# uuwee/Vulkan-PBR-Renderer

Hardware: AMD Instinct MI355X
Metric: IBL-prefilter Mtexels/s (specular prefilter all mips + irradiance; PBR-shaded Mpixels/s under extra.shade_c5 / extra.shade) (higher is better)
Workload: dtype f32; 1 GPU; C4: 4096x4096 specular prefilter (6 faces, 13 mips) + 128x128 irradiance from a 2048^2 HDR cube; env=procedural HDR cube 2048^2 x6 RGBA32F (seed 0x5eed0004, RGBE round-tripped), overlap=False, parallelism=single GPU

## Files before the change

### vulkan-pbr-renderer_amd/csrc/k_mc_region.hip

```cpp
#include "pbr_device.h"
#include "pbr_kernels.h"
#include "k_mc_internal.h"

#include <stdlib.h>
#include <mutex>
#include <type_traits>

typedef float v4f __attribute__((ext_vector_type(4)));
typedef const __attribute__((address_space(4))) v4f* ctab_t;
typedef const __attribute__((address_space(3))) v4f* lds_v4f_p;
typedef const __attribute__((address_space(4))) unsigned* cu32_t;

#define REG_MAX_S 16
#ifndef MC_HEAD_FIRST_SUB
#define MC_HEAD_FIRST_SUB 1
#endif
#ifndef MC_HEAD_FIRST_G1
#define MC_HEAD_FIRST_G1 1
#endif

#ifndef MC_TILE32_SUB
#define MC_TILE32_SUB 1
#endif
#ifndef MC_TILE32_MIN_SIZE
#define MC_TILE32_MIN_SIZE 1024
#endif

struct RegArgs {
    McArgs a;
    int G;
    int RC;
    int NR;
    int NW;
    int expect[REG_MAX_S];
    int pole_row[2];
    const unsigned* tabmax;
    int cut;
    int absorb;
    unsigned long long* stats;
};

__device__ __forceinline__ void face_coords(int f, float x, float y, float z, float& sc, float& tc, float& ma) {
    switch (f) {
    case 0: sc = -z; tc = -y; ma = x; break;
    case 1: sc = z; tc = -y; ma = -x; break;
    case 2: sc = x; tc = z; ma = y; break;
    case 3: sc = x; tc = -z; ma = -y; break;
    case 4: sc = x; tc = -y; ma = z; break;
    default: sc = -x; tc = -y; ma = -z; break;
    }
}

struct RegionView {
    unsigned lds_base;
    f3 Pb, Pt, Pr;
    float half_n, off;
    float ulo, uhi, vlo, vhi;
};

__device__ __forceinline__ void to_face(const v4f e, const RegionView& V, float& sc, float& tc, float& ma) {
    sc = fmaf(e.x, V.Pb.x, fmaf(e.y, V.Pt.x, e.z * V.Pr.x));
    tc = fmaf(e.x, V.Pb.y, fmaf(e.y, V.Pt.y, e.z * V.Pr.y));
    ma = fmaf(e.x, V.Pb.z, fmaf(e.y, V.Pt.z, e.z * V.Pr.z));
}

template <int CLS>
__device__ __forceinline__ void on_face(float sc, float tc, float ma, bool& c1, bool& c2) {
    if (CLS == 0) { c1 = ma > fabsf(sc); c2 = ma > fabsf(tc); }
    else if (CLS == 1) { c1 = ma >= fabsf(sc); c2 = ma > fabsf(tc); }
    else { c1 = ma >= fabsf(sc); c2 = ma >= fabsf(tc); }
}

template <int RS>
__device__ __forceinline__ void tap_accumulate(float w, float u, float v, unsigned lds_base, float& ar, float& ag, float& ab) {
    const int il = (int)u, jl = (int)v;
    const float a = __builtin_amdgcn_fractf(u), b = __builtin_amdgcn_fractf(v);
    unsigned t16, addr;
    asm("v_lshl_add_u32 %0, %1, 4, %2" : "=v"(t16) : "v"(il), "s"(lds_base));
    asm("v_mad_u32_u24 %0, %1, %2, %3" : "=v"(addr) : "v"(jl), "s"(RS * 16), "v"(t16));
    lds_v4f_p tp = (lds_v4f_p)(unsigned long long)addr;
    v4f q00 = tp[0], q10 = tp[1], q01 = tp[RS], q11 = tp[RS + 1];
    asm("" : "+v"(q00)); asm("" : "+v"(q10)); asm("" : "+v"(q01)); asm("" : "+v"(q11));
    const float wa = w * a;
    const float w11 = wa * b;
    const float w10 = wa - w11;
    const float wt = w - wa;
    const float w01 = wt * b;
    const float w00 = wt - w01;
    ar = fmaf(w11, q11.x, fmaf(w01, q01.x, fmaf(w10, q10.x, fmaf(w00, q00.x, ar))));
    ag = fmaf(w11, q11.y, fmaf(w01, q01.y, fmaf(w10, q10.y, fmaf(w00, q00.y, ag))));
    ab = fmaf(w11, q11.z, fmaf(w01, q01.z, fmaf(w10, q10.z, fmaf(w00, q00.z, ab))));
}

template <int RS, bool SUB, int CLS, bool ACC = true>
__device__ __forceinline__ void region_sample(const v4f e, const RegionView& V, float& ar, float& ag, float& ab, unsigned& cnt) {
    float sc, tc, ma;
    to_face(e, V, sc, tc, ma);
    bool c1, c2;
    on_face<CLS>(sc, tc, ma, c1, c2);
    unsigned long long inm = __builtin_amdgcn_ballot_w64(c1) & __builtin_amdgcn_ballot_w64(c2);
    if (inm == 0) return;
    if (!ACC && !SUB) { cnt += (unsigned)__builtin_popcountll(inm); return; }
    bool in = c1 && c2;
    const float h = __builtin_amdgcn_rcpf(ma) * V.half_n;
    const float u = fmaf(sc, h, V.off), v = fmaf(tc, h, V.off);
    if (SUB) {
        const bool c3 = u >= V.ulo, c4 = u < V.uhi, c5 = v >= V.vlo, c6 = v < V.vhi;
        inm &= __builtin_amdgcn_ballot_w64(c3) & __builtin_amdgcn_ballot_w64(c4) & __builtin_amdgcn_ballot_w64(c5) & __builtin_amdgcn_ballot_w64(c6);
        in = in && c3 && c4 && c5 && c6;
    }
    cnt += (unsigned)__builtin_popcountll(inm);
    if (ACC && in) tap_accumulate<RS>(e.w, u, v, V.lds_base, ar, ag, ab);
}

template <int RS>
__device__ __forceinline__ void certain_sample(const v4f e, const RegionView& V, float& ar, float& ag, float& ab) {
    float sc, tc, ma;
    to_face(e, V, sc, tc, ma);
    const float h = __builtin_amdgcn_rcpf(ma) * V.half_n;
    tap_accumulate<RS>(e.w, fmaf(sc, h, V.off), fmaf(tc, h, V.off), V.lds_base, ar, ag, ab);
}

template <int RS, bool SUB, int CLS, bool ACC = true>
__device__ __forceinline__ void lane_sample(const v4f e, const RegionView& V, float& ar, float& ag, float& ab, unsigned& cnt) {
    float sc, tc, ma;
    to_face(e, V, sc, tc, ma);
    bool c1, c2;
    on_face<CLS>(sc, tc, ma, c1, c2);
    bool in = c1 && c2;
    if (SUB && __builtin_amdgcn_ballot_w64(in) == 0ull) return;
    const float h = __builtin_amdgcn_rcpf(ma) * V.half_n;
    const float u = fmaf(sc, h, V.off), v = fmaf(tc, h, V.off);
    if (SUB) in = in && u >= V.ulo && u < V.uhi && v >= V.vlo && v < V.vhi;
    if (in) {
        cnt += 1u;
        if (ACC) tap_accumulate<RS>(e.w, u, v, V.lds_base, ar, ag, ab);
    }
}

template <typename F>
__device__ __forceinline__ void each_sample(unsigned m, ctab_t tw, F&& f) {
    if (m == 0u) return;
    v4f e = tw[__builtin_ctz(m)];
    m &= m - 1u;
    while (m) {
        const v4f en = tw[__builtin_ctz(m)];
        m &= m - 1u;
        f(e);
        e = en;
    }
    f(e);
}

__device__ __forceinline__ float absorb_threshold(float wmax, float m) {
    const float t = wmax * m * 1.00000095367431640625f * 0x1p25f;
    return t < 0x1p-100f ? 0x1p-100f : t;
}

__device__ __forceinline__ void count_absorbed(unsigned* skc, unsigned m, unsigned mu) {
    if (skc && (threadIdx.x & 63) == 0) {
        atomicAdd(&skc[0], 1u);
        atomicAdd(&skc[1], (unsigned)__builtin_popcount(m));
        atomicAdd(&skc[2], (unsigned)__builtin_popcount(mu));
    }
}

template <int RS, bool SUB, int CLS, int REG_S, bool CERT, bool LEAN>
__device__ __forceinline__ void region_pass(const RegionView& V, const unsigned* __restrict__ mwords, const unsigned* __restrict__ cwords, cu32_t wmg,
                                            unsigned rbits, unsigned* skc, int NW, int w0, int w1, ctab_t tab,
                                            float& ar, float& ag, float& ab, unsigned& cnt) {
    unsigned mnext = w0 < w1 ? (unsigned)__builtin_amdgcn_readfirstlane((int)mwords[w0]) : 0u;
    unsigned cnext = (CERT && w0 < w1) ? (unsigned)__builtin_amdgcn_readfirstlane((int)cwords[w0]) : 0u;
    for (int w = w0; w < w1; w += REG_S) {
        unsigned m = mnext;
        unsigned c = cnext;
        mnext = w + REG_S < w1 ? (unsigned)__builtin_amdgcn_readfirstlane((int)mwords[w + REG_S]) : 0u;
        if (CERT) {
            cnext = w + REG_S < w1 ? (unsigned)__builtin_amdgcn_readfirstlane((int)cwords[w + REG_S]) : 0u;
            cnt += 64u * (unsigned)__builtin_popcount(m & c);
        }
        ctab_t tw = tab + (w << 5);
        const unsigned wb = (rbits < 0x7f800000u && m != 0u) ? (LEAN ? wmg[w] : (unsigned)__builtin_amdgcn_readfirstlane((int)cwords[NW + w])) : 0x7f800000u;
        if (wb < 0x7f800000u) {
            const float T = absorb_threshold(__uint_as_float(wb), __uint_as_float(rbits));
            if (__builtin_amdgcn_ballot_w64(!(ar >= T && ag >= T && ab >= T)) == 0ull) {
                if (!CERT) {
                    c = (unsigned)__builtin_amdgcn_readfirstlane((int)cwords[w]);
                    cnt += 64u * (unsigned)__builtin_popcount(m & c);
                }
                count_absorbed(skc, m, m & ~c);
                m &= ~c;
                while (m) {
                    const int i0 = __builtin_ctz(m);
                    m &= m - 1u;
                    region_sample<RS, SUB, CLS, false>(tw[i0], V, ar, ag, ab, cnt);
                }
                continue;
            }
        }
        while (m) {
            const int i0 = __builtin_ctz(m);
            m &= m - 1u;
            const bool two = m != 0u;
            const int i1 = two ? __builtin_ctz(m) : i0;
            m &= m - 1u;
            const v4f e0 = tw[i0];
            const v4f e1 = tw[i1];
            if (CERT && ((c >> i0) & 1u)) certain_sample<RS>(e0, V, ar, ag, ab);
            else region_sample<RS, SUB, CLS>(e0, V, ar, ag, ab, cnt);
            if (two) {
                if (CERT && ((c >> i1) & 1u)) certain_sample<RS>(e1, V, ar, ag, ab);
                else region_sample<RS, SUB, CLS>(e1, V, ar, ag, ab, cnt);
            }
        }
    }
}

template <int RS, bool SUB, int CLS, int REG_S, bool CERT, bool LEAN>
__device__ __forceinline__ void region_pass_runs(const RegionView& V, const unsigned* __restrict__ mwords, const unsigned* __restrict__ cwords, cu32_t wmg,
                                                 unsigned rbits, unsigned* skc, int NW, int s, unsigned long long wsel, ctab_t tab,
                                                 float& ar, float& ag, float& ab, unsigned& cnt) {
    const int wl = s + REG_S * (int)(threadIdx.x & 63);
    unsigned long long nz = __builtin_amdgcn_ballot_w64(wl < NW && mwords[wl] != 0u) & wsel;
    auto tested = [&](const v4f e) { lane_sample<RS, SUB, CLS>(e, V, ar, ag, ab, cnt); };
    while (nz) {
        const int w = s + REG_S * (int)__builtin_ctzll(nz);
        nz &= nz - 1ull;
        const unsigned m = (unsigned)__builtin_amdgcn_readfirstlane((int)mwords[w]);
        unsigned c = CERT ? (unsigned)__builtin_amdgcn_readfirstlane((int)cwords[w]) : 0u;
        ctab_t tw = tab + (w << 5);
        const unsigned wb = rbits < 0x7f800000u ? (LEAN ? wmg[w] : (unsigned)__builtin_amdgcn_readfirstlane((int)cwords[NW + w])) : 0x7f800000u;
        if (wb < 0x7f800000u) {
            const float T = absorb_threshold(__uint_as_float(wb), __uint_as_float(rbits));
            if (__builtin_amdgcn_ballot_w64(!(ar >= T && ag >= T && ab >= T)) == 0ull) {
                if (!CERT) c = (unsigned)__builtin_amdgcn_readfirstlane((int)cwords[w]);
                cnt += (unsigned)__builtin_popcount(m & c);
                count_absorbed(skc, m, m & ~c);
                each_sample(m & ~c, tw, [&](const v4f e) { lane_sample<RS, SUB, CLS, false>(e, V, ar, ag, ab, cnt); });
                continue;
            }
        }
        if (!CERT) { each_sample(m, tw, tested); continue; }
        cnt += (unsigned)__builtin_popcount(m & c);
        unsigned mc = m & c, mu = m & ~c;
        for (;;) {
            const unsigned below = mu ? (mu & (0u - mu)) - 1u : ~0u;
            each_sample(mc & below, tw, [&](const v4f e) { certain_sample<RS>(e, V, ar, ag, ab); });
            mc &= ~below;
            if (!mu) break;
            const int it = __builtin_ctz(mu);
            mu &= mu - 1u;
            tested(tw[it]);
        }
    }
}

template <bool LEAN, bool G1, bool TWO>
__device__ __forceinline__ void region_bin(unsigned* masks, unsigned* any, unsigned* dmax, int NR, int NW, int G, int RC, int n,
                                           f3 R, f3 T, f3 B, f3 Rc, f3 Tc, f3 Bc, ctab_t tab, int n_tab, int tid,
                                           unsigned* cmask, unsigned* wmax, int ntail, int lim, bool keep_cut, int head_end) {
    const float nf = (float)n;
    const float half_n = 0.5f * nf;
    const float off = 0.5f * nf + 0.5f;
    for (int k = tid; k < NR * NW + NR + 1 + ntail; k += 1024) masks[k] = 0u;
    __syncthreads();
    {
        f3 dR = sub3(R, Rc), dT = sub3(T, Tc), dB = sub3(B, Bc);
        float d2 = dot3(dR, dR) + dot3(dT, dT) + dot3(dB, dB);
        atomicMax(dmax, __float_as_uint(sqrtf(d2)));
    }
    __syncthreads();
    const float delta = __uint_as_float(*dmax) * 0.70710678f * 1.001f + 4e-6f;
    const int i_end = (TWO && !keep_cut) ? min(n_tab, lim) : n_tab;
    for (int i = tid; i < i_end; i += 1024) {
        const v4f e = tab[i];
        const int ab = TWO ? (i >= lim ? 2 : (i >= head_end ? 1 : 0)) : 0;
        const float Lx = fmaf(e.x, Bc.x, fmaf(e.y, Tc.x, e.z * Rc.x));
        const float Ly = fmaf(e.x, Bc.y, fmaf(e.y, Tc.y, e.z * Rc.y));
        const float Lz = fmaf(e.x, Bc.z, fmaf(e.y, Tc.z, e.z * Rc.z));
        const unsigned bit = 1u << (i & 31);
        if (!LEAN && wmax) atomicMax(&wmax[i >> 5], __float_as_uint(e.w));
#pragma unroll
        for (int f = 0; f < 6; ++f) {
            float sc, tc, ma;
            face_coords(f, Lx, Ly, Lz, sc, tc, ma);
            const float d2 = 1.41421357f * delta;
            if (!(ma + d2 >= fabsf(sc)) || !(ma + d2 >= fabsf(tc))) continue;
            int lo_u = 0, hi_u = n, lo_v = 0, hi_v = n;
            const float mlo = ma - delta;
            bool certain = false;
            if (mlo > 0.2f) {
                const float rm = LEAN ? __builtin_amdgcn_rcpf(ma) : 1.0f / ma, rl = LEAN ? __builtin_amdgcn_rcpf(mlo) : 1.0f / mlo;
                const float ru = sc * rm, rv = tc * rm;
                const float gu = (fabsf(sc) + delta) * rl, gv = (fabsf(tc) + delta) * rl;
                const float su = fmaf(gu, gu, 1.0f), sv = fmaf(gv, gv, 1.0f);
                const float mu = delta * (LEAN ? __builtin_amdgcn_sqrtf(su) : sqrtf(su)) * rl * half_n * 1.0001f + 0.05f;
                const float mv = delta * (LEAN ? __builtin_amdgcn_sqrtf(sv) : sqrtf(sv)) * rl * half_n * 1.0001f + 0.05f;
                const float uc = fmaf(ru, half_n, off), vc = fmaf(rv, half_n, off);
                const float ul = floorf(uc - mu), uh = floorf(uc + mu), vl = floorf(vc - mv), vh = floorf(vc + mv);
                if (uh < 0.0f || ul > nf || vh < 0.0f || vl > nf) continue;
                lo_u = (int)fmaxf(ul, 0.0f); hi_u = (int)fminf(uh, nf);
                lo_v = (int)fmaxf(vl, 0.0f); hi_v = (int)fminf(vh, nf);
                certain = cmask && ma - d2 > fabsf(sc) && ma - d2 > fabsf(tc) && ul >= 0.0f && uh <= nf && vl >= 0.0f && vh <= nf;
            }
            if (LEAN && G1) {
                if (certain) atomicOr(&cmask[i >> 5], bit);
                atomicOr(&masks[f * NW + (i >> 5)], bit);
                if (TWO) ((unsigned char*)any)[4 * f + ab] = 1;
                else any[f] = 1u;
                continue;
            }
            const int rc = LEAN ? 65 : RC;
            const int gx0 = lo_u / rc, gx1 = hi_u / rc, gy0 = lo_v / rc, gy1 = hi_v / rc;
            if (certain && gx0 == gx1 && gy0 == gy1) atomicOr(&cmask[i >> 5], bit);
            for (int gy = gy0; gy <= gy1; ++gy)
                for (int gx = gx0; gx <= gx1; ++gx) {
                    const int r = (f * G + gy) * G + gx;
                    atomicOr(&masks[r * NW + (i >> 5)], bit);
                    if (TWO) ((unsigned char*)any)[4 * r + ab] = 1;
                    else any[r] = 1u;
                }
        }
    }
}

__device__ __forceinline__ void tile_of_block(const RegArgs& q, int& face, int& tx, int& ty) {
    const McArgs& p = q.a;
    const unsigned tile = blockIdx.x;
    face = p.face0 + (int)(tile / (unsigned)p.tiles_per_face);
    const int tf = (int)(tile % (unsigned)p.tiles_per_face);
    ty = tf / p.tiles_x;
    tx = tf % p.tiles_x;
    if (face < 2) {
        const int ny = p.tiles_per_face / p.tiles_x, pr = q.pole_row[face];
        const int a = min(pr, ny - 1 - pr);
        if (ty <= 2 * a) { const int h = (ty + 1) >> 1; ty = (ty & 1) ? pr + h : pr - h; }
        else { const int rest = ty - 2 * a; ty = (pr > ny - 1 - pr) ? pr - a - rest : pr + a + rest; }
    }
}

template <int TILE>
__device__ __forceinline__ void texel_of_thread(const McArgs& p, int tx, int ty, int t, int& x, int& y) {
    constexpr int QW = TILE / 8, QSH = TILE == 32 ? 2 : 1;
    static_assert(QW == 1 << QSH, "TILE is 16 or 32");
    const int q8 = t >> 6, l8 = t & 63;
    x = tx * TILE + (q8 & (QW - 1)) * 8 + (l8 & 7);
    y = p.y0 + ty * TILE + (q8 >> QSH) * 8 + (l8 >> 3);
}

template <int REG_S, bool RUNS>
__device__ __forceinline__ unsigned cut_credit(int cw, int NW, int n_tab) {
    const int last = NW - 1, kc = (last - cw) / REG_S + 1;
    if (cw > last) return 0u;
    return (unsigned)(32 * kc - ((last - cw) % REG_S == 0 ? 32 * NW - n_tab : 0)) * (RUNS ? 1u : 64u);
}

template <int RS>
__device__ __forceinline__ void stage_rows(float4* region, const float4* __restrict__ fsrc, int nb, int rcx, int rcy, int tid) {
    int tid_s = tid;
    asm volatile("" : "+v"(tid_s));
    const int wv = __builtin_amdgcn_readfirstlane(tid_s >> 6), ln = tid_s & 63;
    const unsigned cx = (unsigned)min(ln, rcx) << 4;
    const char* const base = (const char*)fsrc;
    const unsigned rowb = (unsigned)nb << 4;
    const float4 v0 = *(const float4*)(base + (size_t)((unsigned)min(wv, rcy) * rowb) + cx);
    const float4 v1 = *(const float4*)(base + (size_t)((unsigned)min(wv + 16, rcy) * rowb) + cx);
    const float4 v2 = *(const float4*)(base + (size_t)((unsigned)min(wv + 32, rcy) * rowb) + cx);
    const float4 v3 = *(const float4*)(base + (size_t)((unsigned)min(wv + 48, rcy) * rowb) + cx);
    const float4 v4 = *(const float4*)(base + (size_t)((unsigned)min(wv + 64, rcy) * rowb) + cx);
    const int ey = tid_s >> 1, ex = 64 + (tid_s & 1);
    const float4 ve = *(const float4*)(base + (unsigned)(min(ey, rcy) * nb + min(ex, rcx)) * 16u);
    if (ln <= rcx) {
        float4* const dst = region + wv * RS + ln;
        if (wv <= rcy) dst[0] = v0;
        if (wv + 16 <= rcy) dst[16 * RS] = v1;
        if (wv + 32 <= rcy) dst[32 * RS] = v2;
        if (wv + 48 <= rcy) dst[48 * RS] = v3;
        if (wv + 64 <= rcy) dst[64 * RS] = v4;
    }
    if (tid_s < 2 * RS && ex <= rcx && ey <= rcy) region[ey * RS + ex] = ve;
}

template <int RS, bool MAXIMA>
__device__ __forceinline__ void stage_sweeps(float4* region, const float4* __restrict__ fsrc, int nb, int rcx, int rcy, int tid, unsigned* rmax_r) {
    unsigned vmax = 0u;
    for (int k = tid; k < RS * RS; k += 1024) {
        const int ry = k / RS, rx = k - ry * RS;
        if (rx <= rcx && ry <= rcy) {
            const float4 v = fsrc[ry * nb + rx];
            region[k] = v;
            if (MAXIMA) vmax = max(vmax, max(__float_as_uint(v.x), max(__float_as_uint(v.y), __float_as_uint(v.z))));
        }
    }
    if (MAXIMA && rmax_r) {
        vmax = max(vmax, (unsigned)__builtin_amdgcn_ds_swizzle((int)vmax, (16 << 10) | 0x1f));
        vmax = max(vmax, (unsigned)__builtin_amdgcn_ds_swizzle((int)vmax, (8 << 10) | 0x1f));
        vmax = max(vmax, (unsigned)__builtin_amdgcn_ds_swizzle((int)vmax, (4 << 10) | 0x1f));
        vmax = max(vmax, (unsigned)__builtin_amdgcn_ds_swizzle((int)vmax, (2 << 10) | 0x1f));
        vmax = max(vmax, (unsigned)__builtin_amdgcn_ds_swizzle((int)vmax, (1 << 10) | 0x1f));
        const unsigned wv = max((unsigned)__builtin_amdgcn_readlane((int)vmax, 0), (unsigned)__builtin_amdgcn_readlane((int)vmax, 32));
        if ((tid & 63) == 0) atomicMax(rmax_r, wv);
    }
}

template <int REG_S>
__device__ __forceinline__ void heal_slice(const McArgs& p, ctab_t tab, int NW, int s, f3 R, f3 T, f3 B, float& ar, float& ag, float& ab) {
    const int nb = p.n_src + 2;
    const float nf = (float)p.n_src, off = 0.5f * nf + 0.5f;
    __amdgpu_buffer_rsrc_t rs = __builtin_amdgcn_make_buffer_rsrc((void*)p.src, 0, (int)p.src_bytes, 0x00020000);
    ar = 0.0f; ag = 0.0f; ab = 0.0f;
    for (int w = s; w < NW; w += REG_S) {
        const int i1 = min((w << 5) + 32, p.n_tab);
        for (int i = w << 5; i < i1; ++i) {
            const v4f e = tab[i];
            f3 L;
            L.x = fmaf(e.x, B.x, fmaf(e.y, T.x, e.z * R.x));
            L.y = fmaf(e.x, B.y, fmaf(e.y, T.y, e.z * R.y));
            L.z = fmaf(e.x, B.z, fmaf(e.y, T.z, e.z * R.z));
            f3 c = sample_bordered<false>(rs, L, nf, off, nb, nb * 16);
            ar = fmaf(e.w, c.x, ar); ag = fmaf(e.w, c.y, ag); ab = fmaf(e.w, c.z, ab);
        }
    }
}

template <int REG_TX, int REG_S>
__device__ __forceinline__ void reduce_slices(float* red, int s, int t, float ar, float ag, float ab) {
    red[(s * REG_TX + t) * 3 + 0] = ar;
    red[(s * REG_TX + t) * 3 + 1] = ag;
    red[(s * REG_TX + t) * 3 + 2] = ab;
    __syncthreads();
    for (int stride = REG_S / 2; stride >= 1; stride >>= 1) {
        if (s < stride) {
            const int a2 = (s * REG_TX + t) * 3, b2 = ((s + stride) * REG_TX + t) * 3;
            red[a2 + 0] += red[b2 + 0];
            red[a2 + 1] += red[b2 + 1];
            red[a2 + 2] += red[b2 + 2];
        }
        __syncthreads();
    }
}

#ifdef PBR_MC_PHASE_STAMPS
#define STAMP() ((unsigned long long)__builtin_readcyclecounter())
#else
#define STAMP() 0ull
#endif

template <int RS, bool SUB, int TILE, bool RUNS = false, bool LEAN = false>
__global__ __launch_bounds__(1024) __attribute__((amdgpu_waves_per_eu(8, 8))) void k_mc_region(const RegArgs q) {
    constexpr int REG_TX = TILE * TILE, REG_S = 1024 / REG_TX;
    constexpr bool CERT = SUB;
    constexpr bool ABS = RS == 66;
    const bool absorb_on = ABS && q.absorb;
    constexpr bool OWN_FIRST = ABS;
    constexpr bool TWO = RS == 66 && (SUB ? MC_HEAD_FIRST_SUB != 0 : MC_HEAD_FIRST_G1 != 0);
    const bool cut_on = TWO && LEAN && q.cut != 0;
    extern __shared__ __attribute__((aligned(16))) unsigned char smem_r[];
    float4* region = (float4*)smem_r;
    const unsigned lds_base = (unsigned)(unsigned long long)smem_r;
    unsigned* skc = (unsigned*)(smem_r + RS * RS * 16);
    unsigned* masks = skc + 4;
    unsigned* any = masks + q.NR * q.NW;
    unsigned* dmax = any + q.NR;
    unsigned* cmask = dmax + 1;
    unsigned* wmax = cmask + q.NW;
    unsigned* rmax = wmax + q.NW;
    const int ntail = (absorb_on && !LEAN) ? 2 * q.NW + q.NR : ((CERT || ABS) ? q.NW : 0);
    cu32_t wmg = (cu32_t)(unsigned long long)q.tabmax;
    [[maybe_unused]] const unsigned long long st0 = STAMP();
    const McArgs& p = q.a;
    const int tid = threadIdx.x;
    const int s = __builtin_amdgcn_readfirstlane(tid / REG_TX);
    const int t = tid % REG_TX;

    int face, tx, ty, x, y;
    tile_of_block(q, face, tx, ty);
    texel_of_thread<TILE>(p, tx, ty, t, x, y);
    const int xc = min(x, p.size - 1), yc = min(y, p.y0 + p.rows - 1);

    const f3 R = face_texel_dir(face, xc, yc, p.size);
    const f3 T = tangent_of(R);
    const f3 B = cross3(T, R);
    const f3 Rc = face_texel_dir(face, min(tx * TILE + TILE / 2, p.size - 1), min(p.y0 + ty * TILE + TILE / 2, p.y0 + p.rows - 1), p.size);
    const f3 Tc = tangent_of(Rc);
    const f3 Bc = cross3(Tc, Rc);

    const int n = p.n_src, nb = n + 2;
    const float nf = (float)n;
    const float half_n = 0.5f * nf;
    const float off = 0.5f * nf + 0.5f;
    ctab_t tab = (ctab_t)(unsigned long long)p.tab;
    const int NW = q.NW, NR = q.NR, G = q.G, RC = q.RC;

    if (ABS && tid < 4) skc[tid] = 0u;
    [[maybe_unused]] const unsigned long long st1 = STAMP();
    const int lim = cut_on ? (int)q.tabmax[NW + NR + ((tid >> 5) % REG_S)] << 5 : 0x7fffffff;
    region_bin<LEAN, !SUB, TWO>(masks, any, dmax, NR, NW, G, RC, n, R, T, B, Rc, Tc, Bc, tab, p.n_tab, tid, (CERT || ABS) ? cmask : nullptr,
                                (absorb_on && !LEAN) ? wmax : nullptr, ntail, lim, cut_on && q.stats != nullptr, 32 * REG_S);
    [[maybe_unused]] unsigned long long st_stage = 0ull;
#ifdef PBR_MC_PHASE_STAMPS
    __syncthreads();
#endif
    [[maybe_unused]] const unsigned long long st2 = STAMP();

    float ar = 0.0f, ag = 0.0f, ab = 0.0f;
    unsigned cnt = cut_on ? cut_credit<REG_S, RUNS>((int)wmg[NW + NR + s], NW, p.n_tab) : 0u;
    if (q.stats) {
        __syncthreads();
        unsigned fl = 0, cfl = 0, cwd = 0;
        for (int k = tid; k < NR * NW; k += 1024) {
            const unsigned mk = masks[k];
            fl += __popc(mk);
            if (cut_on) {
                const int w = k % NW;
                if (w >= (int)q.tabmax[NW + NR + (w % REG_S)]) { cfl += __popc(mk); cwd += mk != 0u; masks[k] = 0u; }
            }
        }
        constexpr unsigned BLK = REG_TX / 256;
        if (fl) atomicAdd(&q.stats[2], (unsigned long long)(fl * BLK));
        if (cwd) { atomicAdd(&skc[0], (16u / REG_S) * cwd); atomicAdd(&skc[1], (16u / REG_S) * cfl); }
        if (tid == 0) { atomicAdd(&q.stats[3], (unsigned long long)p.n_tab * BLK); unsigned v = 0; for (int r = 0; r < NR; ++r) v += (any[r] & (TWO ? 0xffffu : ~0u)) != 0u; atomicAdd(&q.stats[4], (unsigned long long)(v * BLK));
                        if (CERT) { unsigned c = 0; for (int k = 0; k < NW; ++k) c += __popc(cmask[k]); atomicAdd(&q.stats[5], (unsigned long long)(c * BLK)); } }
    }
    auto visit = [&](const int r, const int ph) {
        const int f = r / (G * G);
        const int gy = (r / G) % G, gx = r % G;
        const int ox = gx * RC, oy = gy * RC;
        const int rcx = min(RC, n + 1 - ox), rcy = min(RC, n + 1 - oy);
        const float4* __restrict__ fsrc = p.src + ((size_t)f * nb + oy) * nb + ox;
        const unsigned long long sta = STAMP();
        unsigned rbits = 0x7f800000u;
        if (LEAN && RS == 66) stage_rows<RS>(region, fsrc, nb, rcx, rcy, tid);
        else stage_sweeps<RS, ABS && !LEAN>(region, fsrc, nb, rcx, rcy, tid, (absorb_on && !LEAN) ? &rmax[r] : nullptr);
        if (absorb_on && LEAN) rbits = wmg[NW + r];
        __syncthreads();
        if (absorb_on && !LEAN) rbits = (unsigned)__builtin_amdgcn_readfirstlane((int)rmax[r]);
        const unsigned long long stb = STAMP();
        RegionView V;
        V.lds_base = lds_base - (unsigned)(oy * RS + ox) * 16u;
        face_coords(f, B.x, B.y, B.z, V.Pb.x, V.Pb.y, V.Pb.z);
        face_coords(f, T.x, T.y, T.z, V.Pt.x, V.Pt.y, V.Pt.z);
        face_coords(f, R.x, R.y, R.z, V.Pr.x, V.Pr.y, V.Pr.z);
        V.half_n = half_n; V.off = off;
        V.ulo = (float)ox; V.uhi = (float)(ox + rcx); V.vlo = (float)oy; V.vhi = (float)(oy + rcy);
        const unsigned* mw = masks + r * NW;
        unsigned* const sc = (ABS && q.stats) ? skc : nullptr;
        const unsigned long long wsel = TWO ? (ph ? ~1ull : 1ull) : ~0ull;
        const int w0 = (TWO && ph) ? s + REG_S : s, w1 = (TWO && !ph) ? min(NW, s + 1) : NW;
        auto pass = [&](auto cls) {
            constexpr int CLS = decltype(cls)::value;
            if (RUNS) region_pass_runs<RS, SUB, CLS, REG_S, CERT, LEAN>(V, mw, cmask, wmg, rbits, sc, NW, s, wsel, tab, ar, ag, ab, cnt);
            else region_pass<RS, SUB, CLS, REG_S, CERT, LEAN>(V, mw, cmask, wmg, rbits, sc, NW, w0, w1, tab, ar, ag, ab, cnt);
        };
        switch (f >> 1) {
        case 0: pass(std::integral_constant<int, 0>()); break;
        case 1: pass(std::integral_constant<int, 1>()); break;
        default: pass(std::integral_constant<int, 2>()); break;
        }
        st_stage += stb - sta;
    };
    [[maybe_unused]] const unsigned long long st2b = STAMP();
    if (RUNS) __syncthreads();
    for (int kk = 0; kk < (TWO ? 2 * NR : NR); ++kk) {
        const int ph = TWO && kk >= NR, k = kk - (ph ? NR : 0);
        const int r = OWN_FIRST ? mc_region_visit(k, face * (G * G), G * G) : k;
        if (!RUNS) __syncthreads();
        const unsigned av = RUNS ? (unsigned)__builtin_amdgcn_readfirstlane((int)any[r]) : any[r];
        if ((TWO ? (av >> (8 * ph)) & 0xffu : av) == 0u) continue;
        if (RUNS) __syncthreads();
        visit(r, ph);
    }

    [[maybe_unused]] const unsigned long long st3 = STAMP();
    const bool healed = RUNS ? __builtin_amdgcn_ballot_w64(cnt != (unsigned)q.expect[s]) != 0ull : cnt != 64u * (unsigned)q.expect[s];
    if (healed) heal_slice<REG_S>(p, tab, NW, s, R, T, B, ar, ag, ab);
    if (q.stats && (tid & 63) == 0) {
        if (healed) atomicAdd(&q.stats[0], 1ull);
        atomicAdd(&q.stats[1], 1ull);
    }

    __syncthreads();
    if (absorb_on && q.stats && tid < 3 && skc[tid]) atomicAdd(&q.stats[6 + tid], (unsigned long long)skc[tid]);
    float* red = (float*)smem_r;
    reduce_slices<REG_TX, REG_S>(red, s, t, ar, ag, ab);
    int tid_o = tid, x_o, y_o;
    asm volatile("" : "+v"(tid_o));
    const int t_o = tid_o % REG_TX;
    texel_of_thread<TILE>(p, tx, ty, t_o, x_o, y_o);
    if (x_o < p.size && y_o < p.y0 + p.rows && s == 0) {
        float4 o;
        o.x = red[t_o * 3 + 0] / p.divisor; o.y = red[t_o * 3 + 1] / p.divisor; o.z = red[t_o * 3 + 2] / p.divisor; o.w = p.alpha;
        p.out[((size_t)face * p.size + y_o) * p.size + x_o] = o;
    }
#ifdef PBR_MC_PHASE_STAMPS
    if (q.stats && tid == 0) {
        atomicAdd(&q.stats[9], st1 - st0); atomicAdd(&q.stats[10], st2 - st1); atomicAdd(&q.stats[11], st_stage);
        atomicAdd(&q.stats[12], (st3 - st2b) - st_stage); atomicAdd(&q.stats[13], STAMP() - st3);
    }
#endif
}

extern "C" int pbrk_mc_region_order(int face, int G, int k) {
    if (face < 0 || face > 5 || G < 1 || k < 0 || k >= 6 * G * G) return -1;
    return mc_region_visit(k, face * (G * G), G * G);
}

static unsigned long long* g_reg_stats = nullptr;
#define REG_STATS_BYTES 128

static int read_stats(unsigned long long* out, int first_slot, int count) {
    if (!g_reg_stats || !out) return PBRK_E_ARG;
    return hipMemcpy(out, g_reg_stats + first_slot, (size_t)count * 8, hipMemcpyDeviceToHost) == hipSuccess ? PBRK_OK : PBRK_E_LAUNCH;
}
extern "C" int pbrk_mc_region_stats(unsigned long long* out2, int reset) {
    const int rc = read_stats(out2, 0, 2);
    if (rc != PBRK_OK) return rc;
    return (reset && hipMemset(g_reg_stats, 0, REG_STATS_BYTES) != hipSuccess) ? PBRK_E_LAUNCH : PBRK_OK;
}
extern "C" int pbrk_mc_region_skip_stats(unsigned long long* out3) { return read_stats(out3, 6, 3); }
extern "C" int pbrk_mc_region_window_stats(unsigned long long* out1) { return read_stats(out1, 5, 1); }
extern "C" int pbrk_mc_region_flag_stats(unsigned long long* out3) { return read_stats(out3, 2, 3); }
extern "C" int pbrk_mc_region_phase_stats(unsigned long long* out5) { return read_stats(out5, 9, 5); }

template <int RS, bool SUB, int TILE, bool RUNS = false, bool LEAN = false>
static void launch_region_t(const RegArgs& q, unsigned grid, size_t lds, hipStream_t st) {
    static bool attr_set = false;
    if (!attr_set) { (void)hipFuncSetAttribute((const void*)k_mc_region<RS, SUB, TILE, RUNS, LEAN>, hipFuncAttributeMaxDynamicSharedMemorySize, 160 * 1024); attr_set = true; }
    hipLaunchKernelGGL((k_mc_region<RS, SUB, TILE, RUNS, LEAN>), dim3(grid), dim3(1024), lds, st, q);
}

__global__ __launch_bounds__(256) void k_mc_prep(const float4* __restrict__ src, int n, int G, int RC, int NR,
                                                 const float4* __restrict__ tab, int n_tab, int NW, unsigned* __restrict__ out) {
    const int tid = threadIdx.x;
    if ((int)blockIdx.x >= NR) {
        const int w = ((int)blockIdx.x - NR) * 256 + tid;
        if (w >= NW) return;
        unsigned m = 0u;
        for (int i = w << 5; i < min((w << 5) + 32, n_tab); ++i) m = max(m, __float_as_uint(tab[i].w));
        out[w] = m;
        return;
    }
    __shared__ unsigned red, redlo;
    if (tid == 0) { red = 0u; redlo = 0xffffffffu; }
    __syncthreads();
    const int r = (int)blockIdx.x, nb = n + 2;
    const int f = r / (G * G), gy = (r / G) % G, gx = r % G;
    const int ox = gx * RC, oy = gy * RC;
    const int cols = min(RC, n + 1 - ox) + 1, rows = min(RC, n + 1 - oy) + 1;
    const float4* __restrict__ fsrc = src + ((size_t)f * nb + oy) * nb + ox;
    unsigned m = 0u, lo = 0xffffffffu;
    for (int k = tid; k < rows * cols; k += 256) {
        const int ry = k / cols, rx = k - ry * cols;
        const float4 v = fsrc[ry * nb + rx];
        m = max(m, max(__float_as_uint(v.x), max(__float_as_uint(v.y), __float_as_uint(v.z))));
        lo = min(lo, min(__float_as_uint(v.x), min(__float_as_uint(v.y), __float_as_uint(v.z))));
    }
    atomicMax(&red, m);
    atomicMin(&redlo, lo);
    __syncthreads();
    if (tid == 0) { out[NW + r] = red; out[NW + NR + 4 + r] = redlo; }
}

__global__ __launch_bounds__(64) void k_mc_cut(const float4* __restrict__ tab, int n_tab, int NW, int NR, int S, unsigned* __restrict__ out) {
    __shared__ double H[4];
    const int tid = threadIdx.x;
    if (tid < 4) {
        double h = 0.0;
        if (tid < S && NW > S)
            for (int i = 0; i < 32; ++i) h += (double)tab[(tid << 5) + i].w;
        H[tid] = h;
    }
    __syncthreads();
    if (tid != 0) return;
    unsigned M = 0u, m = 0xffffffffu;
    for (int r = 0; r < NR; ++r) { M = max(M, out[NW + r]); m = min(m, out[NW + NR + 4 + r]); }
    int cut4[4];
    mc_launch_cut_s(out, NW, S, H, m, M, cut4);
    for (int s = 0; s < 4; ++s) out[NW + NR + s] = (unsigned)cut4[s % S];
}

extern "C" int pbrk_mc_launch_cut(const float* weights, int n, unsigned min_bits, unsigned max_bits, int* cut4) {
    return pbrk_mc_launch_cut_slices(weights, n, 4, min_bits, max_bits, cut4);
}
extern "C" int pbrk_mc_launch_cut_slices(const float* weights, int n, int S, unsigned min_bits, unsigned max_bits, int* cut4) {
    if (!weights || !cut4 || n < 1 || n > 8192 || (S != 1 && S != 2 && S != 4)) return -1;
    const int NW = (n + 31) / 32;
    unsigned wbits[256];
    for (int w = 0; w < NW; ++w) {
        unsigned m = 0u;
        for (int i = w << 5; i < (w << 5) + 32 && i < n; ++i) {
            union { float f; unsigned u; } c;
            c.f = weights[i];
            m = c.u > m ? c.u : m;
        }
        wbits[w] = m;
    }
    double H[4] = {0.0, 0.0, 0.0, 0.0};
    if (NW > S)
        for (int s = 0; s < S; ++s)
            for (int i = 0; i < 32; ++i) H[s] += (double)weights[(s << 5) + i];
    return mc_launch_cut_s(wbits, NW, S, H, min_bits, max_bits, cut4);
}

#define PREP_SLOTS 32
#define PREP_SLOT_WORDS 4096
#define PREP_MAX_DEVICES 16
struct PrepRing { unsigned* dev; hipEvent_t ev[PREP_SLOTS]; bool used[PREP_SLOTS]; unsigned next; };
static PrepRing g_prep[PREP_MAX_DEVICES];
static std::mutex g_prep_lock;

static unsigned* prep_acquire(hipStream_t st, int* slot_out) {
    hipStreamCaptureStatus cs = hipStreamCaptureStatusNone;
    if (hipStreamIsCapturing(st, &cs) != hipSuccess) { (void)hipGetLastError(); return nullptr; }
    if (cs != hipStreamCaptureStatusNone) return nullptr;
    int dev = 0;
    if (hipGetDevice(&dev) != hipSuccess || dev < 0 || dev >= PREP_MAX_DEVICES) return nullptr;
    PrepRing& R = g_prep[dev];
    if (!R.dev) {
        if (hipMalloc(&R.dev, (size_t)PREP_SLOTS * PREP_SLOT_WORDS * 4) != hipSuccess) { (void)hipGetLastError(); R.dev = nullptr; return nullptr; }
        for (int i = 0; i < PREP_SLOTS; ++i) {
            R.used[i] = false;
            if (hipEventCreateWithFlags(&R.ev[i], hipEventDisableTiming) != hipSuccess) { (void)hipGetLastError(); (void)hipFree(R.dev); R.dev = nullptr; return nullptr; }
        }
        R.next = 0;
    }
    const int slot = (int)(R.next++ % PREP_SLOTS);
    if (R.used[slot] && hipStreamWaitEvent(st, R.ev[slot], 0) != hipSuccess) { (void)hipGetLastError(); return nullptr; }
    *slot_out = slot;
    return R.dev + (size_t)slot * PREP_SLOT_WORDS;
}

int g_mc_region_mode = -1, g_mc_lds_mode = -1;
extern "C" void pbrk_mc_set_kernels(int region, int lds) { g_mc_region_mode = region; g_mc_lds_mode = lds; }
static int g_mc_absorb = 1;
extern "C" void pbrk_mc_set_absorb(int on) { g_mc_absorb = on ? 1 : 0; }
static int g_mc_runs = 1;
extern "C" void pbrk_mc_set_runs(int on) { g_mc_runs = on ? 1 : 0; }
static int g_mc_lean = 1;
extern "C" void pbrk_mc_set_prologue(int lean) { g_mc_lean = lean ? 1 : 0; }

static int g_mc_launch_cut = 1;
extern "C" void pbrk_mc_set_launch_cut(int on) { g_mc_launch_cut = on ? 1 : 0; }
static int g_mc_tile32 = -1;
extern "C" void pbrk_mc_set_tile32(int mode) { g_mc_tile32 = mode < 0 ? -1 : (mode ? 1 : 0); }
static const unsigned* g_last_cut = nullptr;
static int g_last_cut_nw = 0, g_last_cut_s = 4;
extern "C" int pbrk_mc_launch_cut_stats(int* out6) {
    if (!out6) return PBRK_E_ARG;
    const int NW = g_last_cut_nw, S = g_last_cut_s;
    for (int j = 0; j < 4; ++j) { const int s = j % S; out6[j] = s >= NW ? s : s + S * ((NW - s + S - 1) / S); }
    out6[4] = NW; out6[5] = 0;
    if (!g_last_cut) return PBRK_OK;
    if (hipDeviceSynchronize() != hipSuccess) return PBRK_E_LAUNCH;
    int c[4];
    if (hipMemcpy(c, g_last_cut, 16, hipMemcpyDeviceToHost) != hipSuccess) return PBRK_E_LAUNCH;
    for (int s = 0; s < 4; ++s) { if (s < S) out6[5] += (out6[s] - c[s]) / S; out6[s] = c[s]; }
    return PBRK_OK;
}

template <bool SUB, int TILE, bool LEAN>
static void launch_66(const RegArgs& q, unsigned grid, size_t lds, hipStream_t st) {
    if (g_mc_runs) launch_region_t<66, SUB, TILE, true, LEAN>(q, grid, lds, st);
    else launch_region_t<66, SUB, TILE, false, LEAN>(q, grid, lds, st);
}

template <bool LEAN>
static void launch_shape(int RS, int tile, const RegArgs& q, unsigned grid, size_t lds, hipStream_t st) {
    if (tile == 32) launch_66<true, 32, LEAN>(q, grid, lds, st);
    else if (RS == 18) launch_region_t<18, false, 16, false, LEAN>(q, grid, lds, st);
    else if (RS == 34) launch_region_t<34, false, 16, false, LEAN>(q, grid, lds, st);
    else if (q.G == 1) launch_66<false, 16, LEAN>(q, grid, lds, st);
    else launch_66<true, 16, LEAN>(q, grid, lds, st);
}

static bool mc_tile32(int n_src, int n_tab, int size) {
    if (n_src <= 64 || (n_tab + 31) / 32 > 64) return false;
    const int mode = g_mc_tile32 < 0 ? (MC_TILE32_SUB ? -1 : 0) : g_mc_tile32;
    return mode > 0 || (mode < 0 && size >= MC_TILE32_MIN_SIZE);
}

bool launch_mc_region(McArgs a, int nfaces, hipStream_t st) {
    static int stats_on = -1;
    if (g_mc_region_mode < 0) { const char* e = getenv("PBR_MC_REGION"); g_mc_region_mode = e ? atoi(e) : 1; }
    if (!g_mc_region_mode) return false;
    if (a.n_src < 16 || a.size < 256 || a.n_tab < 1 || a.n_tab > 8192) return false;
    RegArgs q;
    q.a = a;
    int RS;
    if (a.n_src <= 16) { RS = 18; q.G = 1; q.RC = a.n_src + 1; }
    else if (a.n_src <= 32) { RS = 34; q.G = 1; q.RC = a.n_src + 1; }
    else if (a.n_src <= 64) { RS = 66; q.G = 1; q.RC = a.n_src + 1; }
    else { RS = 66; q.RC = 65; q.G = (a.n_src + 1 + 64) / 65; }
    q.NR = 6 * q.G * q.G;
    q.NW = (a.n_tab + 31) / 32;
    q.absorb = RS == 66 ? g_mc_absorb : 0;
    const size_t lds_fixed = (size_t)RS * RS * 16 + (4 + (size_t)q.NR * q.NW + q.NR + 1 + q.NW) * 4;
    size_t lds = lds_fixed + (q.absorb ? (size_t)(q.NW + q.NR) * 4 : 0);
    if (lds > 80 * 1024) { q.absorb = 0; lds = lds_fixed; }
    if (lds < (size_t)1024 * 3 * 4) lds = (size_t)1024 * 3 * 4;
    if (lds > 80 * 1024) return false;
    if (stats_on < 0) {
        const char* e = getenv("PBR_MC_STATS"); stats_on = e ? atoi(e) : 0;
        if (stats_on) { if (hipMalloc(&g_reg_stats, REG_STATS_BYTES) != hipSuccess) g_reg_stats = nullptr; else (void)hipMemset(g_reg_stats, 0, REG_STATS_BYTES); }
    }
    q.stats = g_reg_stats;
    const int tile = mc_tile32(a.n_src, a.n_tab, a.size) ? 32 : 16, nslices = 1024 / (tile * tile);
    for (int s = 0; s < REG_MAX_S; ++s) q.expect[s] = 0;
    for (int w = 0; w < q.NW; ++w) { int c = a.n_tab - w * 32; q.expect[w % nslices] += c > 32 ? 32 : c; }
    q.a.tiles_x = (a.size + tile - 1) / tile;
    const int tiles_y = (a.rows + tile - 1) / tile;
    q.a.tiles_per_face = q.a.tiles_x * tiles_y;
    {
        const double vy_vx = 6.11831989512 / 12.123825810901;
        for (int f = 0; f < 2; ++f) {
            int row = (int)((f == 0 ? 0.5 * (1.0 - vy_vx) : 0.5 * (1.0 + vy_vx)) * a.size);
            int tr = (row - a.y0) / tile;
            if (row < a.y0) tr = 0;
            q.pole_row[f] = tr < 0 ? 0 : (tr > tiles_y - 1 ? tiles_y - 1 : tr);
        }
    }
    const unsigned grid = (unsigned)(q.a.tiles_per_face * nfaces);
    bool lean = g_mc_lean != 0;
    q.tabmax = nullptr;
    q.cut = 0;
    g_last_cut = nullptr; g_last_cut_nw = q.NW; g_last_cut_s = nslices;
    if (lean && q.absorb) {
        std::lock_guard<std::mutex> hold(g_prep_lock);
        int slot = -1;
        unsigned* scratch = q.NW + 2 * q.NR + 4 <= PREP_SLOT_WORDS ? prep_acquire(st, &slot) : nullptr;
        if (!scratch) lean = false;
        else {
            int dev = 0; (void)hipGetDevice(&dev);
            q.tabmax = scratch;
            hipLaunchKernelGGL(k_mc_prep, dim3((unsigned)(q.NR + (q.NW + 255) / 256)), dim3(256), 0, st, a.src, a.n_src, q.G, q.RC, q.NR, a.tab, a.n_tab, q.NW, scratch);
            const bool head_first = RS == 66 && (q.G == 1 ? MC_HEAD_FIRST_G1 != 0 : MC_HEAD_FIRST_SUB != 0);
            if (head_first && g_mc_launch_cut && q.NW > nslices) {
                hipLaunchKernelGGL(k_mc_cut, dim3(1), dim3(64), 0, st, a.tab, a.n_tab, q.NW, q.NR, nslices, scratch);
                q.cut = 1;
                g_last_cut = scratch + q.NW + q.NR;
            }
            launch_shape<true>(RS, tile, q, grid, lds, st);
            if (hipEventRecord(g_prep[dev].ev[slot], st) == hipSuccess) g_prep[dev].used[slot] = true;
            return true;
        }
    }
    if (lean) launch_shape<true>(RS, tile, q, grid, lds, st);
    else launch_shape<false>(RS, tile, q, grid, lds, st);
    return true;
}
```

Baseline: 2676 Mtexels/s.

## Enable certain-sample fast path for single-region (G1) and RS=34 run kernels

```diff
diff --git a/vulkan-pbr-renderer_amd/csrc/k_mc_region.hip b/vulkan-pbr-renderer_amd/csrc/k_mc_region.hip
--- a/vulkan-pbr-renderer_amd/csrc/k_mc_region.hip
+++ b/vulkan-pbr-renderer_amd/csrc/k_mc_region.hip
@@ -17,6 +17,9 @@
 #endif
 #ifndef MC_HEAD_FIRST_G1
 #define MC_HEAD_FIRST_G1 1
+#endif
+#ifndef MC_CERT_G1
+#define MC_CERT_G1 1
 #endif
 
 #ifndef MC_TILE32_SUB
@@ -255,7 +258,7 @@
     }
 }
 
-template <bool LEAN, bool G1, bool TWO>
+template <bool LEAN, bool G1, bool TWO, bool PROOF, bool SOLE>
 __device__ __forceinline__ void region_bin(unsigned* masks, unsigned* any, unsigned* dmax, int NR, int NW, int G, int RC, int n,
                                            f3 R, f3 T, f3 B, f3 Rc, f3 Tc, f3 Bc, ctab_t tab, int n_tab, int tid,
                                            unsigned* cmask, unsigned* wmax, int ntail, int lim, bool keep_cut, int head_end) {
@@ -280,6 +283,8 @@
         const float Lz = fmaf(e.x, Bc.z, fmaf(e.y, Tc.z, e.z * Rc.z));
         const unsigned bit = 1u << (i & 31);
         if (!LEAN && wmax) atomicMax(&wmax[i >> 5], __float_as_uint(e.w));
+        [[maybe_unused]] int nflag = 0;
+        [[maybe_unused]] bool proved = false;
 #pragma unroll
         for (int f = 0; f < 6; ++f) {
             float sc, tc, ma;
@@ -301,8 +306,9 @@
                 if (uh < 0.0f || ul > nf || vh < 0.0f || vl > nf) continue;
                 lo_u = (int)fmaxf(ul, 0.0f); hi_u = (int)fminf(uh, nf);
                 lo_v = (int)fmaxf(vl, 0.0f); hi_v = (int)fminf(vh, nf);
-                certain = cmask && ma - d2 > fabsf(sc) && ma - d2 > fabsf(tc) && ul >= 0.0f && uh <= nf && vl >= 0.0f && vh <= nf;
+                certain = PROOF && cmask && ma - d2 > fabsf(sc) && ma - d2 > fabsf(tc) && ul >= 0.0f && uh <= nf && vl >= 0.0f && vh <= nf;
             }
+            if (SOLE) { ++nflag; proved = proved || certain; certain = false; }
             if (LEAN && G1) {
                 if (certain) atomicOr(&cmask[i >> 5], bit);
                 atomicOr(&masks[f * NW + (i >> 5)], bit);
@@ -321,6 +327,7 @@
                     else any[r] = 1u;
                 }
         }
+        if (SOLE && proved && nflag == 1) atomicOr(&cmask[i >> 5], bit);
     }
 }
 
@@ -449,7 +456,7 @@
 template <int RS, bool SUB, int TILE, bool RUNS = false, bool LEAN = false>
 __global__ __launch_bounds__(1024) __attribute__((amdgpu_waves_per_eu(8, 8))) void k_mc_region(const RegArgs q) {
     constexpr int REG_TX = TILE * TILE, REG_S = 1024 / REG_TX;
-    constexpr bool CERT = SUB;
+    constexpr bool CERT = SUB || (RUNS && (RS != 66 || MC_CERT_G1 != 0));
     constexpr bool ABS = RS == 66;
     const bool absorb_on = ABS && q.absorb;
     constexpr bool OWN_FIRST = ABS;
@@ -495,7 +502,7 @@
     if (ABS && tid < 4) skc[tid] = 0u;
     [[maybe_unused]] const unsigned long long st1 = STAMP();
     const int lim = cut_on ? (int)q.tabmax[NW + NR + ((tid >> 5) % REG_S)] << 5 : 0x7fffffff;
-    region_bin<LEAN, !SUB, TWO>(masks, any, dmax, NR, NW, G, RC, n, R, T, B, Rc, Tc, Bc, tab, p.n_tab, tid, (CERT || ABS) ? cmask : nullptr,
+    region_bin<LEAN, !SUB, TWO, CERT || ABS, CERT && !SUB>(masks, any, dmax, NR, NW, G, RC, n, R, T, B, Rc, Tc, Bc, tab, p.n_tab, tid, (CERT || ABS) ? cmask : nullptr,
                                 (absorb_on && !LEAN) ? wmax : nullptr, ntail, lim, cut_on && q.stats != nullptr, 32 * REG_S);
     [[maybe_unused]] unsigned long long st_stage = 0ull;
 #ifdef PBR_MC_PHASE_STAMPS
@@ -758,19 +765,21 @@
     return PBRK_OK;
 }
 
-template <bool SUB, int TILE, bool LEAN>
-static void launch_66(const RegArgs& q, unsigned grid, size_t lds, hipStream_t st) {
-    if (g_mc_runs) launch_region_t<66, SUB, TILE, true, LEAN>(q, grid, lds, st);
-    else launch_region_t<66, SUB, TILE, false, LEAN>(q, grid, lds, st);
+template <int RS, bool SUB, int TILE, bool LEAN, bool HAS_RUNS = true>
+static void launch_runs(const RegArgs& q, unsigned grid, size_t lds, hipStream_t st) {
+    if constexpr (HAS_RUNS) {
+        if (g_mc_runs && q.NW <= 64 * (1024 / (TILE * TILE))) { launch_region_t<RS, SUB, TILE, true, LEAN>(q, grid, lds, st); return; }
+    }
+    launch_region_t<RS, SUB, TILE, false, LEAN>(q, grid, lds, st);
 }
 
 template <bool LEAN>
 static void launch_shape(int RS, int tile, const RegArgs& q, unsigned grid, size_t lds, hipStream_t st) {
-    if (tile == 32) launch_66<true, 32, LEAN>(q, grid, lds, st);
-    else if (RS == 18) launch_region_t<18, false, 16, false, LEAN>(q, grid, lds, st);
-    else if (RS == 34) launch_region_t<34, false, 16, false, LEAN>(q, grid, lds, st);
-    else if (q.G == 1) launch_66<false, 16, LEAN>(q, grid, lds, st);
-    else launch_66<true, 16, LEAN>(q, grid, lds, st);
+    if (tile == 32) launch_runs<66, true, 32, LEAN>(q, grid, lds, st);
+    else if (RS == 18) launch_runs<18, false, 16, LEAN, false>(q, grid, lds, st);
+    else if (RS == 34) launch_runs<34, false, 16, LEAN>(q, grid, lds, st);
+    else if (q.G == 1) launch_runs<66, false, 16, LEAN>(q, grid, lds, st);
+    else launch_runs<66, true, 16, LEAN>(q, grid, lds, st);
 }
 
 static bool mc_tile32(int n_src, int n_tab, int size) {
```

Measured after the change: 2749 Mtexels/s (median of 6 runs). 1.03x the previous value.
